# mala-lab/GGAD

Measured on AMD Instinct MI355X. Metric: training nodes/sec (DGraph-Fin mini-batch GGAD), higher is better.
Workload: dtype f32; 1 GPU; DGraph-Fin-size synthetic graph, mini-batch GGAD (GCN encoder); nodes=3700550, directed_entries=72953930, feat=17, emb=64, batch=150+50, graph=powerlaw(alpha=2.1,max_degree=2000), chunk_batches=150, hop2=ldsw, overlap=False, dense_cus=0, chain=0, dense_steps=XCD-resident chunk kernel: one launch per chunk on 28 CUs of one XCD, parallelism=dp1, optimizer=adam(lr=1e-3,wd=0.007), batch_streams=the reference's stream

## Files before the change

ggad_amd/csrc/common.h:

```cpp
#pragma once
#include <hip/hip_runtime.h>
#include <stdint.h>
#include <mutex>
#include "../../include/ggad_hip.h"

#define GGAD_WAVE 64
#define GGAD_MAX_D 64
#define GGAD_MAX_F 1024

void ggad_set_error(hipError_t e, const char *where);

#define GGAD_CHECK_LAUNCH(where)                 \
  do {                                           \
    hipError_t _e = hipGetLastError();           \
    if (_e != hipSuccess) {                      \
      ggad_set_error(_e, where);                 \
      return GGAD_E_LAUNCH;                      \
    }                                            \
  } while (0)

#define GGAD_REQUIRE(cond) \
  do {                     \
    if (!(cond)) return GGAD_E_INVALID; \
  } while (0)
// ... 32 lines not shown

__device__ __forceinline__ void ggad_adam_elem(float &pi, float &mi, float &vi, float g, float wd, float sc0, float sc1) {
  float gi = fmaf(wd, pi, g);
  mi = fmaf(gi - mi, 0.1f, mi);
  vi = fmaf(0.001f * gi, gi, vi * 0.999f);
  const float denom = sqrtf(vi) / sc1 + 1e-8f;
  pi = pi - sc0 * (mi / denom);
}

__device__ __forceinline__ int lower_bound_i32(const int32_t *__restrict__ a, int lo, int hi, int key) {
  while (lo < hi) {
    int mid = (lo + hi) >> 1;
    if (a[mid] < key) lo = mid + 1; else hi = mid;
  }
  return lo;
}

__device__ __forceinline__ bool ggad_vblock(int skip, unsigned &vb, unsigned &vg) {
  const unsigned b = blockIdx.x, n = gridDim.x;
  if (skip < 0) { vb = b; vg = n; return true; }
  const unsigned sk = (unsigned)skip;
  if ((b & 7u) == sk) return false;
  vb = b - ((b >> 3) + ((b & 7u) > sk ? 1u : 0u));
  vg = n - ((n >> 3) + ((n & 7u) > sk ? 1u : 0u));
  return true;
}
static inline unsigned ggad_skip_grid(unsigned want, int skip) { return skip < 0 ? want : (unsigned)(((uint64_t)(want + 1) * 8 + 6) / 7); }

constexpr int GGAD_CTR_STRIDE = 16;
constexpr int GGAD_CTR_GROUPS = 0 * GGAD_CTR_STRIDE, GGAD_CTR_ITEMS = 1 * GGAD_CTR_STRIDE, GGAD_CTR_PART = 2 * GGAD_CTR_STRIDE,
              GGAD_CTR_CURSOR = 3 * GGAD_CTR_STRIDE, GGAD_CTR_PC = 4 * GGAD_CTR_STRIDE,
              GGAD_CTR_BIG = 5 * GGAD_CTR_STRIDE,
              GGAD_CTR_RANGE0 = 6 * GGAD_CTR_STRIDE,
              GGAD_CTR_PROF = 14 * GGAD_CTR_STRIDE;
constexpr int GGAD_RANGES = 8;
constexpr int GGAD_RANGE_DEG = 256;
constexpr int GGAD_PLAN_COUNTERS = 16 * GGAD_CTR_STRIDE;

struct ggad_plan_view {
  const int32_t *batch_ptr, *batch_ent_ptr, *nodes, *row_slot, *ent_ptr, *row_ck_ptr, *ck_rc, *ck_e0;
  int32_t n_batches, n_rows, n_ents, n_chunks;
  int32_t seg_stride;
  int64_t pair_bound;
};
int ggad_int_hop1(const ggad_mb_plan *P, const ggad_plan_view &V, int ldsw, int reset_now, hipStream_t st);
int ggad_int_global_hop2(const ggad_mb_plan *P, const ggad_plan_view &V, hipStream_t st, hipEvent_t ev0, hipEvent_t ev1);
int ggad_int_ldsw_hop2(const ggad_mb_plan *P, const ggad_plan_view &V, hipStream_t st, hipEvent_t ev0, hipEvent_t ev1);
int ggad_int_range_deg();

int ggad_int_gemm_slab(const float *A, const float *B, float *C, int M, int N, int K, int64_t lda, int64_t sbk, int64_t sbn, int64_t ldc,
                       const float *bias, int relu, hipStream_t st, const float *prelu_a = nullptr, float *C2 = nullptr, int64_t ldc2 = 0);

int64_t ggad_int_wgrad_tn_ws(int R, int m, int n);
int ggad_int_wgrad_tn(const float *P, int64_t ldp, const float *Q, int64_t ldq, int R, int m, int n, float *D, float *ws, hipStream_t st,
                      int *vpq = nullptr);

constexpr int GGAD_MB_BWD_PARTS = 256;
struct ggad_xchg_view;
bool ggad_int_wide_ok(int D, int F);
int ggad_int_wide_project(const float *params, int32_t D, int32_t F, const float *x2, const int32_t *ent_own, int32_t ent0,
                          int32_t n_ents, float *h2, ggad_stream_t stream);
int ggad_int_wide_fwd_rows(const float *params, int32_t D, int32_t F, const float *x1, const float *h2, const int32_t *ent_ptr,
                           const int32_t *ent_own, const int32_t *labels, int32_t row0, int32_t n_rows, int32_t ent0, float *h1,
                           float *nbar, float *gen, ggad_stream_t stream);
int ggad_int_wide_loss(const float *params, int32_t D, int32_t F, const float *h1, const float *nbar, const float *gen,
                       const int32_t *labels, const int32_t *pos_meta, const int32_t *row_pos, const int32_t *ent_ptr,
                       int32_t row0, int32_t n_rows, float *loss_ws, float *losses8, float *d_h1, float *d_gen, float *d_nbar,
                       float *dz, float *coef_a, float *coef_g, int32_t *step_counter, ggad_stream_t stream);
int ggad_int_wide_row_coefs(const float *params, int32_t D, int32_t F, const int32_t *labels, const int32_t *ent_ptr,
                            int32_t row0, int32_t n_rows, const float *h1, const float *gen, const float *d_h1,
// ... 29 lines not shown
```

ggad_amd/csrc/hop2_ldsw.hip:

```cpp
#include <algorithm>
#include <atomic>
#include <climits>
#include <mutex>

#include "common.h"

namespace {

#ifdef GGAD_G2_PROF
struct G2Prof { unsigned long long a[8], t; };
#define G2_ARG , G2Prof &prof
#define G2_PASS , prof
#define G2_MARK(i) do { __builtin_amdgcn_sched_barrier(0); __builtin_amdgcn_s_waitcnt(0); const unsigned long long t_ = wall_clock64(); \
                        prof.a[i] += t_ - prof.t; prof.t = t_; __builtin_amdgcn_sched_barrier(0); } while (0)
#define TC_MARK(i) do { __syncthreads(); if (threadIdx.x == 0) { const unsigned long long t_ = wall_clock64(); tcp[i] += t_ - tct; tct = t_; } } while (0)
#else
#define G2_ARG
#define G2_PASS
#define G2_MARK(i)
#define TC_MARK(i)
#endif

constexpr int SLICE = 256;
constexpr int GRP_W = 10;
// ... 503 lines not shown
      for (int q = 0; q < 4; ++q) wa[4 * c + q] = a < G ? wv[q] : 0.0f;
    }
    __builtin_amdgcn_wave_barrier();
    {
      const int ix = min(blk + 64 + lane, last);
      k_nx = col[s + ix];
#pragma unroll
      for (int j = 0; j < G; ++j) c_nx[j] = pc[pb[j] + ix];
    }
    G2_MARK(3);
#pragma unroll
    for (int i = 0; i < 16; ++i) {
      acc0 = __builtin_amdgcn_mfma_f32_16x16x4f32(wa[i], x[i].x, acc0, 0, 0, 0);
      acc1 = __builtin_amdgcn_mfma_f32_16x16x4f32(wa[i], x[i].y, acc1, 0, 0, 0);
    }
    G2_MARK(4);
  }
#pragma unroll
  for (int j = 0; j < G; ++j) {
    const int src = (lane >> 1) + 16 * (j >> 2);
    const float v0 = __shfl(acc0[j & 3], src & 63, GGAD_WAVE), v1 = __shfl(acc1[j & 3], src & 63, GGAD_WAVE);
    tot[j] = (lane & 1) ? v1 : v0;
  }
}

__device__ __forceinline__ int range_tile(int r, int n_tiles) { return (int)(((int64_t)r * n_tiles) / GGAD_RANGES); }

__global__ void __launch_bounds__(256) k_build_groups(const int32_t *__restrict__ ent_own, const int32_t *__restrict__ ent_col,
                                                      const int32_t *__restrict__ own_deg, int n_ents,
                                                      int32_t *__restrict__ node_head, const int32_t *__restrict__ own_next,
                                                      const int32_t *__restrict__ tile_off, int n_tiles,
                                                      int32_t *__restrict__ grp, int32_t *__restrict__ items,
                                                      int32_t *__restrict__ big, int32_t *__restrict__ gbnd,
                                                      int32_t *__restrict__ counters, int range_deg, int skip) {
  unsigned vbx, vgx;
  if (!ggad_vblock(skip, vbx, vgx)) return;
  const int e = vbx * 256 + threadIdx.x;
  const int lane = lane_id();
  int u = 0, m = 0, ng = 0, ns = 0, deg = 0;
  if (e < n_ents && ent_own[e] == e) {
    u = ent_col[e];
    if (node_head[u] == e + 1) {
      for (int cur = e + 1; cur != 0; cur = own_next[cur - 1]) ++m;
      ng = (m + 7) >> 3;
      deg = own_deg[e];
      ns = deg > range_deg ? GGAD_RANGES : (deg > SLICE ? (deg + SLICE - 1) / SLICE : 1);
    }
  }
  const bool is_big = deg > range_deg;
  const int c1 = is_big ? 0 : ng * ns, c2 = ns > 1 ? m * ns : 0, c3 = is_big ? ng : 0;
  int v0 = ng, v1 = c1, v2 = c2, v3 = c3;
#pragma unroll
  for (int off = 1; off < GGAD_WAVE; off <<= 1) {
    const int t0 = __shfl_up(v0, off, GGAD_WAVE), t1 = __shfl_up(v1, off, GGAD_WAVE), t2 = __shfl_up(v2, off, GGAD_WAVE),
              t3 = __shfl_up(v3, off, GGAD_WAVE);
    if (lane >= off) { v0 += t0; v1 += t1; v2 += t2; v3 += t3; }
  }
  __shared__ int wg_tot[4][5];
  const int wid = threadIdx.x >> 6;
  if (lane == GGAD_WAVE - 1) { wg_tot[0][wid] = v0; wg_tot[1][wid] = v1; wg_tot[2][wid] = v2; wg_tot[3][wid] = v3; }
  __syncthreads();
  if (threadIdx.x < 4) {
    const int k = threadIdx.x;
    int sum = 0;
    for (int w = 0; w < 4; ++w) { const int t = wg_tot[k][w]; wg_tot[k][w] = sum; sum += t; }
    int32_t *ctr = counters + (k == 0 ? GGAD_CTR_GROUPS : (k == 1 ? GGAD_CTR_ITEMS : (k == 2 ? GGAD_CTR_PART : GGAD_CTR_BIG)));
    wg_tot[k][4] = sum > 0 ? atomicAdd(ctr, sum) : 0;
  }
  __syncthreads();
  const int b0 = wg_tot[0][4] + wg_tot[0][wid], b1 = wg_tot[1][4] + wg_tot[1][wid], b2 = wg_tot[2][4] + wg_tot[2][wid],
            b3 = wg_tot[3][4] + wg_tot[3][wid];
  if (ng == 0) return;
  const int gbase = b0 + v0 - ng, ibase = b1 + v1 - c1, pbase = b2 + v2 - c2, bbase = b3 + v3 - c3;
  int bnd[GGAD_RANGES + 1];
  if (is_big) {
    const int32_t *row = tile_off + (int64_t)u * (n_tiles + 1);
#pragma unroll
    for (int r = 0; r <= GGAD_RANGES; ++r) bnd[r] = row[range_tile(r, n_tiles)];
  }
  int cur = e + 1;
  for (int g = 0; g < ng; ++g) {
    int32_t *rec = grp + (int64_t)(gbase + g) * GRP_W;
#pragma unroll
    for (int j = 0; j < 8; ++j) {
      int v = -1;
      if (cur != 0) { v = cur - 1; cur = own_next[v]; }
      rec[j] = v;
    }
    rec[8] = pbase + g * 8 * ns;
    rec[9] = ns;
    if (is_big) {
      big[bbase + g] = gbase + g;
      int32_t *bo = gbnd + (int64_t)(bbase + g) * (GGAD_RANGES + 1);
#pragma unroll
      for (int r = 0; r <= GGAD_RANGES; ++r) bo[r] = bnd[r];
    } else {
      for (int sl = 0; sl < ns; ++sl) {
        int32_t *it = items + (int64_t)(ibase + sl * ng + g) * 2;
        it[0] = gbase + g;
        it[1] = sl;
      }
    }
  }
  node_head[u] = 0;
}

template <int FT, bool MF>
__global__ void __launch_bounds__(256) k_gather2_items(const int32_t *__restrict__ col, const float *__restrict__ feat, int F_rt,
                                                       int stride, const int32_t *__restrict__ own_rp,
                                                       const int32_t *__restrict__ own_deg, const int32_t *__restrict__ pw_base,
                                                       const uint16_t *__restrict__ pc, const int32_t *__restrict__ grp,
                                                       const int32_t *__restrict__ items, const int32_t *__restrict__ big,
                                                       const int32_t *__restrict__ gbnd, int32_t *__restrict__ counters,
                                                       float *__restrict__ x2, float *__restrict__ part2, int affine, int take_cap, int skip) {
  static_assert(ITEM_GRAB == 4 && GRP_W <= 10, "lane layout of the metadata loads: 16 lanes per item of a grab (10, 11: range bounds)");
  unsigned vbx, vgx;
  if (!ggad_vblock(skip, vbx, vgx)) return;
  const int F = FT ? FT : F_rt;
  const int lane = lane_id();
  __shared__ __attribute__((aligned(16))) float mf_lds[MF ? 4 * MF_LDS : 4];
  float *lw = mf_lds + (MF ? (threadIdx.x >> 6) * MF_LDS : 0);
  const int n_small = counters[GGAD_CTR_ITEMS], n_big = counters[GGAD_CTR_BIG];
  const int q_l = lane >> 4, r_l = lane & 15;
// ... 81 lines not shown
        else if (n == 2) { float t2[2]; gather_slice_mfma<2>(col, feat, s, n0, n1, inv_sr, n, pb, pc, lane, lw, k_first, t2 G2_PASS); tot[0] = t2[0]; tot[1] = t2[1]; }
        else if (n <= 4) { float t4[4]; gather_slice_mfma<4>(col, feat, s, n0, n1, inv_sr, n, pb, pc, lane, lw, k_first, t4 G2_PASS);
#pragma unroll
          for (int j = 0; j < 4; ++j) tot[j] = t4[j]; }
        else gather_slice_mfma<8>(col, feat, s, n0, n1, inv_sr, n, pb, pc, lane, lw, k_first, tot G2_PASS);
      } else
      if (n == 1) { float t1[1]; gather_slice<1, FT>(col, feat, F, stride, s, n0, n1, inv_sr, n, pb, pc, lane, k_first, t1 G2_PASS); tot[0] = t1[0]; }
      else if (n == 2) { float t2[2]; gather_slice<2, FT>(col, feat, F, stride, s, n0, n1, inv_sr, n, pb, pc, lane, k_first, t2 G2_PASS); tot[0] = t2[0]; tot[1] = t2[1]; }
      else if (n <= 4) { float t4[4]; gather_slice<4, FT>(col, feat, F, stride, s, n0, n1, inv_sr, n, pb, pc, lane, k_first, t4 G2_PASS);
#pragma unroll
        for (int j = 0; j < 4; ++j) tot[j] = t4[j]; }
      else gather_slice<8, FT>(col, feat, F, stride, s, n0, n1, inv_sr, n, pb, pc, lane, k_first, tot G2_PASS);
#pragma unroll
      for (int j = 0; j < 8; ++j) {
        if (j < n && lane < F) {
          if (ns == 1) x2[(int64_t)e[j] * F + lane] = (deg == 0) ? inv_sr * 0.0f : tot[j];
          else part2[((int64_t)pbase + (int64_t)j * ns + sl) * F + lane] = tot[j];
        }
      }
      G2_MARK(5);
    }
    }
  }
  }
#ifdef GGAD_G2_PROF
  if (lane == 0) {
    prof.a[6] = wall_clock64() - t_begin;
    unsigned long long *out = reinterpret_cast<unsigned long long *>(counters + GGAD_CTR_PROF);
    for (int k = 0; k < 7; ++k) atomicAdd(out + k, prof.a[k]);
  }
#endif
}

__global__ void __launch_bounds__(256) k_gather2_combine(const int32_t *__restrict__ grp, const int32_t *__restrict__ counters,
                                                         const float *__restrict__ part2, int F, float *__restrict__ x2, int skip) {
  unsigned vbx, vgx;
  if (!ggad_vblock(skip, vbx, vgx)) return;
  const int lane = lane_id();
  const int n_groups = counters[GGAD_CTR_GROUPS];
  const int rpi = 64 / F;
  const int g = lane / F, f = lane - g * F;
  for (int gi = vbx * 4 + (threadIdx.x >> 6); gi < n_groups; gi += vgx * 4) {
    const int rv = (lane < GRP_W) ? grp[(int64_t)gi * GRP_W + lane] : -1;
    const int ns = __builtin_amdgcn_readlane(rv, 9);
    if (ns <= 1) continue;
    const int pbase = __builtin_amdgcn_readlane(rv, 8);
    for (int j0 = 0; j0 < 8; j0 += rpi) {
      const int j = j0 + g;
      const int ej = __shfl(rv, j & 7, GGAD_WAVE);
      if (g < rpi && j < 8 && ej >= 0) {
        float acc = 0.0f;
#pragma unroll 4
        for (int sl = 0; sl < ns; ++sl) acc += part2[((int64_t)pbase + (int64_t)j * ns + sl) * F + f];
        x2[(int64_t)ej * F + f] = acc;
      }
    }
  }
}

__global__ void __launch_bounds__(256) k_gather2_w(const int32_t *__restrict__ col, const float *__restrict__ feat, int F, int stride,
                                                   const int32_t *__restrict__ ent_own, int n_ents,
                                                   const int32_t *__restrict__ own_rp, const int32_t *__restrict__ own_deg,
                                                   const int32_t *__restrict__ pw_base, const uint16_t *__restrict__ pc,
                                                   float *__restrict__ x2, int skip) {
  unsigned vbx, vgx;
  if (!ggad_vblock(skip, vbx, vgx)) return;
  const int e0 = vbx * 4 + (threadIdx.x >> 6);
  if (e0 >= n_ents || ent_own[e0] != e0) return;
  const int lane = lane_id();
  const int s = own_rp[e0];
  const int deg = own_deg[e0];
  const int pb0 = pw_base[e0];
  const float inv_sr = 1.0f / sqrtf((float)deg);
  if (F <= 64) {
    const int pb[8] = {pb0, 0, 0, 0, 0, 0, 0, 0};
    float total = 0.0f;
#ifdef GGAD_G2_PROF
    G2Prof prof = {};
// ... 47 lines not shown
  const int n_tiles = (int)((P->n_nodes + TW_TILE - 1) >> TW_SHIFT);
  const int skip = P->xcd_skip >= 0 && P->xcd_skip < 8 ? P->xcd_skip : -1;
  const bool tile_major = P->tile_start != nullptr && P->col_t != nullptr;
  k_seg_transpose<<<dim3(ggad_skip_grid((unsigned)((V.n_ents + 63) / 64), skip)), dim3(256), 0, st>>>(
      P->tile_off, tile_major ? P->tile_start : nullptr, n_tiles, P->ent_own, P->ent_col, V.n_ents, V.seg_stride, P->seg_t, skip);
  const size_t lds = (size_t)(TW_TILE / 2) * 4 + (size_t)(3 * TW_MAXOWN + 1) * 4 + (size_t)TW_BRK * 4;
  {
    static std::mutex mu;
    static int state[64] = {};
    int dev = 0;
    if (hipGetDevice(&dev) != hipSuccess || dev < 0 || dev >= 64) return GGAD_E_INVALID;
    std::lock_guard<std::mutex> lock(mu);
    if (state[dev] == 0) {
      const bool ok = hipFuncSetAttribute((const void *)k_tile_counts, hipFuncAttributeMaxDynamicSharedMemorySize, (int)lds) == hipSuccess;
      (void)hipGetLastError();
      state[dev] = ok ? 1 : -1;
    }
    if (state[dev] != 1) { ggad_set_error(hipErrorInvalidValue, "mb_plan_build: this device cannot give k_tile_counts its LDS"); return GGAD_E_LAUNCH; }
  }
  if (P->ev_tile0) (void)hipEventRecord(static_cast<hipEvent_t>(P->ev_tile0), st);
  static const int tc_map = [] { const char *e = getenv("GGAD_TC_MAP"); return e ? atoi(e) : -1; }();
  const bool class_map = tc_map >= 0 ? tc_map != 0 : tile_major;
  const unsigned tc_grid = class_map ? 8u * (unsigned)((n_tiles + (skip < 0 ? 8 : 7) - 1) / (skip < 0 ? 8 : 7)) * (unsigned)V.n_batches
                                      : ggad_skip_grid((unsigned)n_tiles * (unsigned)V.n_batches, skip);
  k_tile_counts<<<dim3(tc_grid), dim3(TW_T), lds, st>>>(tile_major ? P->col_t : P->col, P->seg_t, V.seg_stride, P->own_rp, V.batch_ent_ptr,
                                                        P->pw_base, P->pc, n_tiles, V.n_batches, P->counters, skip, (tile_major ? 1 : 0) | (class_map ? 2 : 0));
  if (P->ev_tile1) (void)hipEventRecord(static_cast<hipEvent_t>(P->ev_tile1), st);
  if (ev0) (void)hipEventRecord(ev0, st);
  const int F = P->feat_dim;
  if (P->node_major && F <= 64) {
    const int range_deg = ggad_int_range_deg();
    static const int affine = [] { const char *e = getenv("GGAD_RANGE_AFFINE"); return e ? atoi(e) : 1; }();
    int32_t *big = P->items + 2 * (int64_t)P->item_cap, *gbnd = P->items + 3 * (int64_t)P->item_cap;
    k_build_groups<<<dim3(ggad_skip_grid((unsigned)((V.n_ents + 255) / 256), skip)), dim3(256), 0, st>>>(
        P->ent_own, P->ent_col, P->own_deg, V.n_ents, P->node_head, P->own_next, P->tile_off, n_tiles, P->grp, P->items, big, gbnd,
        P->counters, range_deg, skip);
    const int64_t max_items = (int64_t)V.n_ents + (V.pair_bound > 0 ? V.pair_bound : P->pair_cap) / SLICE;
    static const int env_wg = [] { const char *e = getenv("GGAD_G2_WG_PER_CU"); return e ? atoi(e) : 0; }();
    static const int env_cap = [] { const char *e = getenv("GGAD_G2_TAKE_CAP"); return e ? atoi(e) : 0; }();
    const bool small_launch = V.n_batches <= 32;
    const int wg_per_cu = env_wg > 0 ? env_wg : (small_launch ? 3 : 4);
    const int take_cap = env_cap > 0 ? env_cap : (small_launch ? 8 : 12);
    const unsigned wgs = (unsigned)std::min<int64_t>((max_items + 4 * ITEM_GRAB - 1) / (4 * ITEM_GRAB), 256 * wg_per_cu);
    if (F == 17 && P->feat_stride == 32 && V.n_batches >= g_mfma_batches.load())
      k_gather2_items<17, true><<<dim3(ggad_skip_grid(wgs, skip)), dim3(256), 0, st>>>(P->col, P->feat, F, P->feat_stride, P->own_rp, P->own_deg,
                                                                                       P->pw_base, P->pc, P->grp, P->items, big, gbnd, P->counters,
                                                                                       P->x2, P->part2, affine, take_cap, skip);
    else if (F == 17)
      k_gather2_items<17, false><<<dim3(ggad_skip_grid(wgs, skip)), dim3(256), 0, st>>>(P->col, P->feat, F, P->feat_stride, P->own_rp, P->own_deg,
                                                                                 P->pw_base, P->pc, P->grp, P->items, big, gbnd, P->counters,
                                                                                 P->x2, P->part2, affine, take_cap, skip);
    else
      k_gather2_items<0, false><<<dim3(ggad_skip_grid(wgs, skip)), dim3(256), 0, st>>>(P->col, P->feat, F, P->feat_stride, P->own_rp, P->own_deg,
                                                                                P->pw_base, P->pc, P->grp, P->items, big, gbnd, P->counters,
                                                                                P->x2, P->part2, affine, take_cap, skip);
    const unsigned cg = (unsigned)std::min<int64_t>(((int64_t)V.n_ents + 3) / 4, 16384);
    k_gather2_combine<<<dim3(ggad_skip_grid(cg, skip)), dim3(256), 0, st>>>(P->grp, P->counters, P->part2, F, P->x2, skip);
  } else {
    k_gather2_w<<<dim3(ggad_skip_grid((unsigned)((V.n_ents + 3) / 4), skip)), dim3(256), 0, st>>>(
        P->col, P->feat, F, P->feat_stride, P->ent_own, V.n_ents, P->own_rp, P->own_deg, P->pw_base, P->pc, P->x2, skip);
  }
  if (ev1) (void)hipEventRecord(ev1, st);
  GGAD_CHECK_LAUNCH("mb_plan_build (ldsw 2-hop)");
  return GGAD_OK;
}

extern "C" {

int ggad_mb_ldsw_tile_shift(void) { return TW_SHIFT; }
int ggad_mb_ldsw_max_owners(void) { return TW_MAXOWN; }
int32_t ggad_mb_slice_len(void) { return SLICE; }
int32_t ggad_mb_group_words(void) { return GRP_W; }
int ggad_mb_set_gather_options(int32_t mfma_min_batches, int32_t range_deg) {
  if (mfma_min_batches >= 0) g_mfma_batches.store(mfma_min_batches);
  if (range_deg >= 0) g_range_deg.store(range_deg);
  return GGAD_OK;
}
int32_t ggad_mb_item_words(void) { return 3 + GGAD_RANGES + 1; }
int32_t ggad_mb_plan_counter_elems(void) { return GGAD_PLAN_COUNTERS; }
int64_t ggad_mb_tile_offsets_elems(int64_t n_nodes, int32_t tile_shift) {
  return n_nodes * (((n_nodes + (1LL << tile_shift) - 1) >> tile_shift) + 1);
}
int64_t ggad_mb_ldsw_seg_elems(int64_t n_nodes, int64_t n_entries_cap) {
  return 2 * (((n_nodes + TW_TILE - 1) >> TW_SHIFT) + 1) * ((n_entries_cap + 63) / 64 * 64);
}

int ggad_mb_tile_offsets(const int32_t *rowptr, const int32_t *col, int64_t n_nodes, int32_t tile_shift, int32_t *tile_off,
                         ggad_stream_t stream) {
  GGAD_REQUIRE(rowptr && col && tile_off && n_nodes >= 0 && tile_shift >= 8 && tile_shift <= 24);
  if (n_nodes == 0) return GGAD_OK;
// ... 32 lines not shown
```

ggad_amd/csrc/plan.hip:

```cpp
#include "common.h"

namespace {

constexpr int SCAN_T = 256;
constexpr int SCAN_ITEMS = 8;
constexpr int SCAN_TILE = SCAN_T * SCAN_ITEMS;

__device__ __forceinline__ int block_exclusive_scan(int v, int *total) {
  __shared__ int wsum[SCAN_T / GGAD_WAVE];
  const int lane = lane_id(), wid = threadIdx.x / GGAD_WAVE;
  int inc = v;
#pragma unroll
  for (int off = 1; off < GGAD_WAVE; off <<= 1) {
    int t = __shfl_up(inc, off, GGAD_WAVE);
    if (lane >= off) inc += t;
  }
  if (lane == GGAD_WAVE - 1) wsum[wid] = inc;
  __syncthreads();
  int base = 0, tot = 0;
#pragma unroll
  for (int w = 0; w < SCAN_T / GGAD_WAVE; ++w) {
    int s = wsum[w];
    if (w < wid) base += s;
    tot += s;
// ... 51 lines not shown
      const int jj = __shfl(j, src & 63, GGAD_WAVE);
      const float ws = __shfl(w, src & 63, GGAD_WAVE);
      ww[u] = (src < count) ? ws : 0.0f;
      x[u] = (lane_active && src < count) ? feat[(int64_t)jj * F + fbase + f] : 0.0f;
    }
#pragma unroll
    for (int u = 0; u < 4; ++u) acc = fmaf(ww[u], x[u], acc);
  }
  for (; t < iters; ++t) {
    const int src = t * rpi + g;
    const int jj = __shfl(j, src & 63, GGAD_WAVE);
    const float ws = __shfl(w, src & 63, GGAD_WAVE);
    const float ww = (src < count) ? ws : 0.0f;
    const float x = (lane_active && src < count) ? feat[(int64_t)jj * F + fbase + f] : 0.0f;
    acc = fmaf(ww, x, acc);
  }
}

__device__ __forceinline__ float reduce_groups(float acc, int F, int rpi) {
  float tot = acc;
  for (int gg = 1; gg < rpi; ++gg) tot += __shfl(acc, (lane_id() + gg * F) & 63, GGAD_WAVE);
  return tot;
}

__global__ void __launch_bounds__(256) k_expand(const int32_t *__restrict__ rowptr, const int32_t *__restrict__ col,
                                                const int32_t *__restrict__ nodes, const int32_t *__restrict__ row_slot,
                                                const int32_t *__restrict__ ent_ptr, const int32_t *__restrict__ ck_rc,
                                                const int32_t *__restrict__ ck_e0, int n_chunks, int64_t n_nodes,
                                                int32_t *__restrict__ ent_col, int32_t *__restrict__ ent_slot,
                                                int32_t *__restrict__ ent_row, int32_t *__restrict__ cnt1,
                                                int32_t *__restrict__ own1, int32_t *__restrict__ counters, int skip) {
  unsigned vbx, vgx;
  if (!ggad_vblock(skip, vbx, vgx)) return;
  if (vbx == 0 && threadIdx.x < GGAD_PLAN_COUNTERS && counters != nullptr) counters[threadIdx.x] = 0;
  const int ck = (int)((vbx * 256u + threadIdx.x) >> 4);
  const int i = threadIdx.x & 15;
  if (ck >= n_chunks) return;
  const int rc = ck_rc[ck];
  if (i >= (rc & 63)) return;
  const int row = rc >> 6;
  const int e = ck_e0[ck] + i;
  const int e_row = ent_ptr[row];
  const int r = ent_ptr[row + 1] - e_row;
  const int idx = e - e_row;
  const int v = nodes[row];
  const int s = rowptr[v];
  const int deg = rowptr[v + 1] - s;
  int j;
  if (r == deg) {
    j = col[s + idx];
  } else {
    const int a = idx > 0 ? col[s + idx - 1] : -1;
    const int b = idx < deg ? col[s + idx] : 0x7fffffff;
    j = (b < v) ? b : (a < v ? v : a);
  }
  const int slot = row_slot[row];
  ent_col[e] = j;
  ent_slot[e] = slot;
  ent_row[e] = row;
  const int64_t soff = (int64_t)slot * n_nodes;
  const int old = atomicAdd(&cnt1[soff + j], 1);
  if (old == 0) own1[soff + j] = e;
}

__global__ void __launch_bounds__(256) k_gather1c(const float *__restrict__ feat, int F, int stride,
                                                  const int32_t *__restrict__ row_slot, const int32_t *__restrict__ ent_ptr,
                                                  const int32_t *__restrict__ row_ck_ptr, const int32_t *__restrict__ ck_rc,
// ... 370 lines not shown
```

ggad_amd/csrc/plan_build.cpp:

```cpp
#include <algorithm>
#include <chrono>
#include <cstdint>
#include <cstdio>
#include <cstdlib>
#include <cstring>
#include <vector>

#include "common.h"

namespace {
inline int64_t align4(int64_t x) { return (x + 3) & ~(int64_t)3; }
}

extern "C" {

int ggad_event_create(int32_t timing, void **out) {
  if (!out) return GGAD_E_INVALID;
  hipEvent_t ev = nullptr;
  const hipError_t e = hipEventCreateWithFlags(&ev, timing ? hipEventDefault : hipEventDisableTiming);
  if (e != hipSuccess) { ggad_set_error(e, "event_create"); return GGAD_E_LAUNCH; }
  *out = ev;
  return GGAD_OK;
}
int ggad_event_destroy(void *event) {
  if (!event) return GGAD_OK;
  const hipError_t e = hipEventDestroy(static_cast<hipEvent_t>(event));
  if (e != hipSuccess) { ggad_set_error(e, "event_destroy"); return GGAD_E_LAUNCH; }
  return GGAD_OK;
}
int ggad_event_record(void *event, ggad_stream_t stream) {
  if (!event) return GGAD_E_INVALID;
  const hipError_t e = hipEventRecord(static_cast<hipEvent_t>(event), as_stream(stream));
  if (e != hipSuccess) { ggad_set_error(e, "event_record"); return GGAD_E_LAUNCH; }
  return GGAD_OK;
}
int ggad_event_synchronize(void *event) {
  if (!event) return GGAD_E_INVALID;
  const hipError_t e = hipEventSynchronize(static_cast<hipEvent_t>(event));
  if (e != hipSuccess) { ggad_set_error(e, "event_synchronize"); return GGAD_E_LAUNCH; }
  return GGAD_OK;
}
int ggad_event_elapsed_ms(void *start, void *stop, float *ms_host) {
  if (!start || !stop || !ms_host) return GGAD_E_INVALID;
  const hipError_t e = hipEventElapsedTime(ms_host, static_cast<hipEvent_t>(start), static_cast<hipEvent_t>(stop));
  if (e != hipSuccess) { ggad_set_error(e, "event_elapsed_ms"); return GGAD_E_LAUNCH; }
  return GGAD_OK;
}

int ggad_mb_plan_build(const ggad_mb_plan *P, const int64_t *nodes_host, const int32_t *batch_ptr_host, int32_t n_batches,
                       const int64_t *labels_host, ggad_mb_plan_info *info, int64_t *ent_ptr_host_out,
                       int64_t *batch_ent_ptr_host_out, int32_t *batch_max_row_host_out, ggad_stream_t stream) {
  GGAD_REQUIRE(P && nodes_host && batch_ptr_host && info);
  GGAD_REQUIRE(P->rowptr && P->col && P->feat && P->closed_deg_host && P->stage_host && P->stage && P->stage_event);
  GGAD_REQUIRE(P->cnt1 && P->own1 && P->ent_col && P->ent_slot && P->ent_row && P->ent_own && P->ent_c1 && P->x1 && P->ck_part);
  GGAD_REQUIRE(P->feat_dim >= 1 && P->feat_dim <= GGAD_MAX_F && P->feat_stride >= P->feat_dim && P->n_nodes >= 1);
  GGAD_REQUIRE(P->ck_part_stride >= (P->feat_dim < 64 ? 64 : P->feat_dim));
  GGAD_REQUIRE(n_batches >= 1 && n_batches <= P->max_batches && batch_ptr_host[0] == 0);
  const bool train = P->train != 0;
  if (train) GGAD_REQUIRE(labels_host && P->x2 && (P->hop2 == 1 || P->hop2 == 2));
  std::memset(info, 0, sizeof(*info));
  static const bool timing = getenv("GGAD_BUILD_TIMING") != nullptr;
  const auto tt0 = std::chrono::steady_clock::now();
  const int nb = n_batches;
  const int64_t rows = batch_ptr_host[nb];
  GGAD_REQUIRE(rows >= 1 && rows < (1 << 25));
  for (int b = 0; b < nb; ++b) GGAD_REQUIRE(batch_ptr_host[b + 1] > batch_ptr_host[b]);
  const int CL = 16;
  const int SL = ggad_mb_slice_len();

  int64_t n_ents = 0, n_chunks = 0, bound = 0;
  int64_t max_batch_ents = 0;
  const bool want_ldsw = train && P->hop2 == 1;
  if (want_ldsw) GGAD_REQUIRE(P->pair_bound_host && P->tile_off && P->own_deg && P->own_rp && P->pw_base && P->node_head &&
                              P->own_next && P->grp && P->counters);
  static thread_local std::vector<int32_t> row_deg;
  if ((int64_t)row_deg.size() < rows) row_deg.resize((size_t)rows);
  constexpr int PF = 24;
  const int64_t *pack = P->node_pack_host;
  constexpr int64_t PACK_MASK = (1LL << 40) - 1;
  for (int64_t i = 0; i < rows && i < PF; ++i) {
    const int64_t v = nodes_host[i];
    GGAD_REQUIRE(v >= 0 && v < P->n_nodes);
    if (pack) { __builtin_prefetch(&pack[v]); continue; }
    __builtin_prefetch(&P->closed_deg_host[v]);
    if (want_ldsw) __builtin_prefetch(&P->pair_bound_host[v]);
  }
  for (int b = 0; b < nb; ++b) {
    int64_t be = 0;
    for (int64_t i = batch_ptr_host[b]; i < batch_ptr_host[b + 1]; ++i) {
      if (i + PF < rows) {
        const int64_t vn = nodes_host[i + PF];
        GGAD_REQUIRE(vn >= 0 && vn < P->n_nodes);
        if (pack) __builtin_prefetch(&pack[vn]);
        else {
          __builtin_prefetch(&P->closed_deg_host[vn]);
          if (want_ldsw) __builtin_prefetch(&P->pair_bound_host[vn]);
        }
      }
      const int64_t v = nodes_host[i];
      const int64_t pk = pack ? pack[v] : 0;
      const int64_t r = pack ? (pk >> 40) : P->closed_deg_host[v];
      row_deg[(size_t)i] = (int32_t)r;
      be += r;
      n_chunks += (r + CL - 1) / CL;
      if (want_ldsw) bound += pack ? (pk & PACK_MASK) : P->pair_bound_host[v];
    }
    n_ents += be;
    max_batch_ents = std::max(max_batch_ents, be);
  }
  GGAD_REQUIRE(n_ents < (1LL << 31) - 1);
  int mode = train ? P->hop2 : 0;
  if (mode == 1 && (max_batch_ents >= 65536 || bound >= (1LL << 31) - 1 || P->n_nodes * (int64_t)P->feat_stride * 4 >= (1LL << 32)))
    mode = 2;
  const int64_t off_bp = 0, off_bep = align4(nb + 1), off_nodes = off_bep + align4(nb + 1), off_labels = off_nodes + align4(rows),
                off_meta = off_labels + align4(rows), off_rpos = off_meta + align4(rows), off_slot = off_rpos + align4(rows),
                off_eptr = off_slot + align4(rows), off_ckp = off_eptr + align4(rows + 1), off_ckrc = off_ckp + align4(rows + 1),
                off_cke0 = off_ckrc + align4(n_chunks), stage_need = off_cke0 + align4(n_chunks);
  const int64_t seg_stride = (n_ents + 63) / 64 * 64;
  const int64_t n_tiles1 = ((P->n_nodes + (1LL << ggad_mb_ldsw_tile_shift()) - 1) >> ggad_mb_ldsw_tile_shift()) + 1;
  info->pair_bound = bound;
  info->n_batches = nb;
  info->n_rows = (int32_t)rows;
  info->n_ents = (int32_t)n_ents;
  info->n_chunks = (int32_t)n_chunks;
  info->mode = mode;
  info->off_batch_ptr = off_bp; info->off_batch_ent_ptr = off_bep; info->off_nodes = off_nodes; info->off_labels = off_labels;
  info->off_pos_meta = off_meta; info->off_row_pos = off_rpos; info->off_row_slot = off_slot; info->off_ent_ptr = off_eptr;
  info->off_row_ck_ptr = off_ckp; info->off_ck_rc = off_ckrc; info->off_ck_e0 = off_cke0;
  info->need_rows = rows; info->need_ents = n_ents; info->need_chunks = n_chunks; info->need_stage = stage_need;
  if (mode == 1) {
    info->need_pairs = bound;
    info->need_items = n_ents + bound / SL;
    info->need_part2 = (2 + (ggad_int_range_deg() == INT32_MAX ? 0 : (int64_t)GGAD_RANGES * SL / GGAD_RANGE_DEG)) * (bound / SL) + 8;
    info->need_seg = ((P->tile_start && P->col_t) ? 2 : 1) * n_tiles1 * seg_stride;
  }
  info->need_cnt2 = (mode == 2 && P->cnt2 == nullptr) ? 1 : 0;
  if (rows > P->rows_cap || n_ents > P->ent_cap || n_chunks > P->ck_cap || stage_need > P->stage_cap || info->need_cnt2 ||
      (mode == 1 && (info->need_pairs > P->pair_cap || info->need_items > P->item_cap || info->need_part2 > P->part2_cap ||
                     info->need_seg > P->seg_cap)))
    return GGAD_E_CAPACITY;
  if (mode == 1) GGAD_REQUIRE(P->seg_t && P->pc && P->items && P->part2);

  const auto tt1 = std::chrono::steady_clock::now();
  hipStream_t st = as_stream(stream);
  hipError_t he = hipEventSynchronize(static_cast<hipEvent_t>(P->stage_event));
  if (he != hipSuccess) { ggad_set_error(he, "mb_plan_build (stage event)"); return GGAD_E_LAUNCH; }
  const auto tt2 = std::chrono::steady_clock::now();
  int32_t *S = P->stage_host;
  int32_t *bp = S + off_bp, *bep = S + off_bep, *nd = S + off_nodes, *lb = S + off_labels, *meta = S + off_meta,
          *rpos = S + off_rpos, *slot = S + off_slot, *eptr = S + off_eptr, *ckp = S + off_ckp, *ckrc = S + off_ckrc,
          *cke0 = S + off_cke0;
  int64_t e = 0, c = 0;
  for (int b = 0; b < nb; ++b) {
    const int r0 = batch_ptr_host[b], r1 = batch_ptr_host[b + 1];
    bp[b] = r0;
    bep[b] = (int32_t)e;
    if (batch_ent_ptr_host_out) batch_ent_ptr_host_out[b] = e;
    int max_r = 0;
    for (int i = r0; i < r1; ++i) {
      const int32_t v = (int32_t)nodes_host[i];
      const int r = row_deg[(size_t)i];
      nd[i] = v;
      slot[i] = b;
      eptr[i] = (int32_t)e;
      ckp[i] = (int32_t)c;
      if (ent_ptr_host_out) ent_ptr_host_out[i] = e;
      for (int k = 0; k < r; k += CL) {
        ckrc[c] = (i << 6) | std::min(CL, r - k);
        cke0[c] = (int32_t)(e + k);
        ++c;
      }
      e += r;
      max_r = std::max(max_r, r);
    }
    if (batch_max_row_host_out) batch_max_row_host_out[b] = max_r;
    if (train) {
      int q = 0;
      for (int pass = 0; pass < 2; ++pass)
        for (int i = r0; i < r1; ++i) {
          const int64_t l = labels_host[i];
          if (l != 0 && l != 1) return GGAD_E_INVALID;
          if ((int)l != pass) continue;
          meta[r0 + q] = (i << 2) | ((int)l << 1);
          rpos[i] = q;
          ++q;
        }
      for (int i = r0; i < r1; ++i) {
        lb[i] = (int32_t)labels_host[i];
        meta[i] |= (int32_t)labels_host[i];
      }
    }
  }
  bp[nb] = (int32_t)rows;
  bep[nb] = (int32_t)e;
  eptr[rows] = (int32_t)e;
  ckp[rows] = (int32_t)c;
  if (batch_ent_ptr_host_out) batch_ent_ptr_host_out[nb] = e;
  if (ent_ptr_host_out) ent_ptr_host_out[rows] = e;
  const auto tt3 = std::chrono::steady_clock::now();
  he = hipMemcpyAsync(P->stage, S, (size_t)stage_need * sizeof(int32_t), hipMemcpyHostToDevice, st);
  if (he != hipSuccess) { ggad_set_error(he, "mb_plan_build (upload)"); return GGAD_E_LAUNCH; }
  he = hipEventRecord(static_cast<hipEvent_t>(P->stage_event), st);
  if (he != hipSuccess) { ggad_set_error(he, "mb_plan_build (stage event record)"); return GGAD_E_LAUNCH; }

  const auto tt4 = std::chrono::steady_clock::now();
  ggad_plan_view V;
  const int32_t *D = P->stage;
  V.batch_ptr = D + off_bp; V.batch_ent_ptr = D + off_bep; V.nodes = D + off_nodes; V.row_slot = D + off_slot;
  V.ent_ptr = D + off_eptr; V.row_ck_ptr = D + off_ckp; V.ck_rc = D + off_ckrc; V.ck_e0 = D + off_cke0;
  V.n_batches = nb; V.n_rows = (int32_t)rows; V.n_ents = (int32_t)n_ents; V.n_chunks = (int32_t)n_chunks;
  V.seg_stride = (int32_t)seg_stride;
  V.pair_bound = bound;
  int rc = ggad_int_hop1(P, V, mode == 1 ? 1 : 0, mode != 2 ? 1 : 0, st);
  if (rc) return rc;
  hipEvent_t ev0 = static_cast<hipEvent_t>(P->ev_gather0), ev1 = static_cast<hipEvent_t>(P->ev_gather1);
  if (mode == 1) rc = ggad_int_ldsw_hop2(P, V, st, ev0, ev1);
  else if (mode == 2) rc = ggad_int_global_hop2(P, V, st, ev0, ev1);
  if (timing) {
    const auto tt5 = std::chrono::steady_clock::now();
    auto us = [](auto a, auto b) { return std::chrono::duration<double, std::micro>(b - a).count(); };
    fprintf(stderr, "[ggad_mb_plan_build] %d batches: sizes %.1f  stage-event wait %.1f  fill %.1f  copy + event %.1f  launches %.1f us (%lld KB staged)\n", nb,
            us(tt0, tt1), us(tt1, tt2), us(tt2, tt3), us(tt3, tt4), us(tt4, tt5), (long long)(stage_need * 4 / 1024));
  }
  return rc;
}

}
```

Measured before the change: 3.326 million nodes/s.

## Fuse host plan size pass with fill and compact multi-slice combine list

The host plan builder now computes per-row degrees and writes the structural tables in one pass after waiting on the stage event, instead of a size pass followed by a fill pass. Chunk start offsets go to a provisional far location and are moved into place once the chunk count is known. Label partitioning also changes from two scans to a count-then-place pass. On the GPU, group building now records a compact list of groups split across several slices, so the combine kernel walks only those on a smaller grid rather than scanning every group and skipping single-slice ones. The trade-offs are an extra counter slot and item-buffer region, a memmove on the host, and the stage-event wait now happening before the size computation.

```diff
diff --git a/ggad_amd/csrc/common.h b/ggad_amd/csrc/common.h
--- a/ggad_amd/csrc/common.h
+++ b/ggad_amd/csrc/common.h
@@ -88,10 +88,11 @@
               GGAD_CTR_CURSOR = 3 * GGAD_CTR_STRIDE, GGAD_CTR_PC = 4 * GGAD_CTR_STRIDE,
               GGAD_CTR_BIG = 5 * GGAD_CTR_STRIDE,
               GGAD_CTR_RANGE0 = 6 * GGAD_CTR_STRIDE,
-              GGAD_CTR_PROF = 14 * GGAD_CTR_STRIDE;
+              GGAD_CTR_PROF = 14 * GGAD_CTR_STRIDE,
+              GGAD_CTR_MULTI = 16 * GGAD_CTR_STRIDE;
 constexpr int GGAD_RANGES = 8;
 constexpr int GGAD_RANGE_DEG = 256;
-constexpr int GGAD_PLAN_COUNTERS = 16 * GGAD_CTR_STRIDE;
+constexpr int GGAD_PLAN_COUNTERS = 17 * GGAD_CTR_STRIDE;
 
 struct ggad_plan_view {
   const int32_t *batch_ptr, *batch_ent_ptr, *nodes, *row_slot, *ent_ptr, *row_ck_ptr, *ck_rc, *ck_e0;
diff --git a/ggad_amd/csrc/hop2_ldsw.hip b/ggad_amd/csrc/hop2_ldsw.hip
--- a/ggad_amd/csrc/hop2_ldsw.hip
+++ b/ggad_amd/csrc/hop2_ldsw.hip
@@ -559,7 +559,8 @@
                                                       const int32_t *__restrict__ tile_off, int n_tiles,
                                                       int32_t *__restrict__ grp, int32_t *__restrict__ items,
                                                       int32_t *__restrict__ big, int32_t *__restrict__ gbnd,
-                                                      int32_t *__restrict__ counters, int range_deg, int skip) {
+                                                      int32_t *__restrict__ multi, int32_t *__restrict__ counters, int range_deg,
+                                                      int skip) {
   unsigned vbx, vgx;
   if (!ggad_vblock(skip, vbx, vgx)) return;
   const int e = vbx * 256 + threadIdx.x;
@@ -576,29 +577,30 @@
   }
   const bool is_big = deg > range_deg;
   const int c1 = is_big ? 0 : ng * ns, c2 = ns > 1 ? m * ns : 0, c3 = is_big ? ng : 0;
-  int v0 = ng, v1 = c1, v2 = c2, v3 = c3;
+  const int c4 = ns > 1 ? ng : 0;
+  int v0 = ng, v1 = c1, v2 = c2, v3 = c3, v4 = c4;
 #pragma unroll
   for (int off = 1; off < GGAD_WAVE; off <<= 1) {
     const int t0 = __shfl_up(v0, off, GGAD_WAVE), t1 = __shfl_up(v1, off, GGAD_WAVE), t2 = __shfl_up(v2, off, GGAD_WAVE),
-              t3 = __shfl_up(v3, off, GGAD_WAVE);
-    if (lane >= off) { v0 += t0; v1 += t1; v2 += t2; v3 += t3; }
-  }
-  __shared__ int wg_tot[4][5];
+              t3 = __shfl_up(v3, off, GGAD_WAVE), t4 = __shfl_up(v4, off, GGAD_WAVE);
+    if (lane >= off) { v0 += t0; v1 += t1; v2 += t2; v3 += t3; v4 += t4; }
+  }
+  __shared__ int wg_tot[5][5];
   const int wid = threadIdx.x >> 6;
-  if (lane == GGAD_WAVE - 1) { wg_tot[0][wid] = v0; wg_tot[1][wid] = v1; wg_tot[2][wid] = v2; wg_tot[3][wid] = v3; }
+  if (lane == GGAD_WAVE - 1) { wg_tot[0][wid] = v0; wg_tot[1][wid] = v1; wg_tot[2][wid] = v2; wg_tot[3][wid] = v3; wg_tot[4][wid] = v4; }
   __syncthreads();
-  if (threadIdx.x < 4) {
+  if (threadIdx.x < 5) {
     const int k = threadIdx.x;
     int sum = 0;
     for (int w = 0; w < 4; ++w) { const int t = wg_tot[k][w]; wg_tot[k][w] = sum; sum += t; }
-    int32_t *ctr = counters + (k == 0 ? GGAD_CTR_GROUPS : (k == 1 ? GGAD_CTR_ITEMS : (k == 2 ? GGAD_CTR_PART : GGAD_CTR_BIG)));
+    int32_t *ctr = counters + (k == 0 ? GGAD_CTR_GROUPS : (k == 1 ? GGAD_CTR_ITEMS : (k == 2 ? GGAD_CTR_PART : (k == 3 ? GGAD_CTR_BIG : GGAD_CTR_MULTI))));
     wg_tot[k][4] = sum > 0 ? atomicAdd(ctr, sum) : 0;
   }
   __syncthreads();
   const int b0 = wg_tot[0][4] + wg_tot[0][wid], b1 = wg_tot[1][4] + wg_tot[1][wid], b2 = wg_tot[2][4] + wg_tot[2][wid],
-            b3 = wg_tot[3][4] + wg_tot[3][wid];
+            b3 = wg_tot[3][4] + wg_tot[3][wid], b4 = wg_tot[4][4] + wg_tot[4][wid];
   if (ng == 0) return;
-  const int gbase = b0 + v0 - ng, ibase = b1 + v1 - c1, pbase = b2 + v2 - c2, bbase = b3 + v3 - c3;
+  const int gbase = b0 + v0 - ng, ibase = b1 + v1 - c1, pbase = b2 + v2 - c2, bbase = b3 + v3 - c3, mbase = b4 + v4 - c4;
   int bnd[GGAD_RANGES + 1];
   if (is_big) {
     const int32_t *row = tile_off + (int64_t)u * (n_tiles + 1);
@@ -616,6 +618,7 @@
     }
     rec[8] = pbase + g * 8 * ns;
     rec[9] = ns;
+    if (ns > 1) multi[mbase + g] = gbase + g;
     if (is_big) {
       big[bbase + g] = gbase + g;
       int32_t *bo = gbnd + (int64_t)(bbase + g) * (GGAD_RANGES + 1);
@@ -763,18 +766,21 @@
 #endif
 }
 
-__global__ void __launch_bounds__(256) k_gather2_combine(const int32_t *__restrict__ grp, const int32_t *__restrict__ counters,
-                                                         const float *__restrict__ part2, int F, float *__restrict__ x2, int skip) {
+__global__ void __launch_bounds__(256) k_gather2_combine(const int32_t *__restrict__ grp, const int32_t *__restrict__ multi,
+                                                         const int32_t *__restrict__ counters, const float *__restrict__ part2, int F,
+                                                         float *__restrict__ x2, int skip) {
   unsigned vbx, vgx;
   if (!ggad_vblock(skip, vbx, vgx)) return;
+  const int n_multi = counters[GGAD_CTR_MULTI];
+  const int w0 = vbx * 4 + (threadIdx.x >> 6);
+  if (w0 >= n_multi) return;
   const int lane = lane_id();
-  const int n_groups = counters[GGAD_CTR_GROUPS];
   const int rpi = 64 / F;
   const int g = lane / F, f = lane - g * F;
-  for (int gi = vbx * 4 + (threadIdx.x >> 6); gi < n_groups; gi += vgx * 4) {
+  for (int mi = w0; mi < n_multi; mi += vgx * 4) {
+    const int gi = multi[mi];
     const int rv = (lane < GRP_W) ? grp[(int64_t)gi * GRP_W + lane] : -1;
     const int ns = __builtin_amdgcn_readlane(rv, 9);
-    if (ns <= 1) continue;
     const int pbase = __builtin_amdgcn_readlane(rv, 8);
     for (int j0 = 0; j0 < 8; j0 += rpi) {
       const int j = j0 + g;
@@ -888,9 +894,10 @@
     const int range_deg = ggad_int_range_deg();
     static const int affine = [] { const char *e = getenv("GGAD_RANGE_AFFINE"); return e ? atoi(e) : 1; }();
     int32_t *big = P->items + 2 * (int64_t)P->item_cap, *gbnd = P->items + 3 * (int64_t)P->item_cap;
+    int32_t *multi = P->items + (int64_t)(3 + GGAD_RANGES) * P->item_cap;
     k_build_groups<<<dim3(ggad_skip_grid((unsigned)((V.n_ents + 255) / 256), skip)), dim3(256), 0, st>>>(
         P->ent_own, P->ent_col, P->own_deg, V.n_ents, P->node_head, P->own_next, P->tile_off, n_tiles, P->grp, P->items, big, gbnd,
-        P->counters, range_deg, skip);
+        multi, P->counters, range_deg, skip);
     const int64_t max_items = (int64_t)V.n_ents + (V.pair_bound > 0 ? V.pair_bound : P->pair_cap) / SLICE;
     static const int env_wg = [] { const char *e = getenv("GGAD_G2_WG_PER_CU"); return e ? atoi(e) : 0; }();
     static const int env_cap = [] { const char *e = getenv("GGAD_G2_TAKE_CAP"); return e ? atoi(e) : 0; }();
@@ -910,8 +917,9 @@
       k_gather2_items<0, false><<<dim3(ggad_skip_grid(wgs, skip)), dim3(256), 0, st>>>(P->col, P->feat, F, P->feat_stride, P->own_rp, P->own_deg,
                                                                                 P->pw_base, P->pc, P->grp, P->items, big, gbnd, P->counters,
                                                                                 P->x2, P->part2, affine, take_cap, skip);
-    const unsigned cg = (unsigned)std::min<int64_t>(((int64_t)V.n_ents + 3) / 4, 16384);
-    k_gather2_combine<<<dim3(ggad_skip_grid(cg, skip)), dim3(256), 0, st>>>(P->grp, P->counters, P->part2, F, P->x2, skip);
+    const int64_t max_multi = std::min<int64_t>(V.n_ents, (V.pair_bound > 0 ? V.pair_bound : P->pair_cap) / SLICE);
+    const unsigned cg = (unsigned)std::max<int64_t>(1, std::min<int64_t>((max_multi + 3) / 4, 2048));
+    k_gather2_combine<<<dim3(ggad_skip_grid(cg, skip)), dim3(256), 0, st>>>(P->grp, multi, P->counters, P->part2, F, P->x2, skip);
   } else {
     k_gather2_w<<<dim3(ggad_skip_grid((unsigned)((V.n_ents + 3) / 4), skip)), dim3(256), 0, st>>>(
         P->col, P->feat, F, P->feat_stride, P->ent_own, V.n_ents, P->own_rp, P->own_deg, P->pw_base, P->pc, P->x2, skip);
diff --git a/ggad_amd/csrc/plan.hip b/ggad_amd/csrc/plan.hip
--- a/ggad_amd/csrc/plan.hip
+++ b/ggad_amd/csrc/plan.hip
@@ -107,7 +107,8 @@
                                                 int32_t *__restrict__ own1, int32_t *__restrict__ counters, int skip) {
   unsigned vbx, vgx;
   if (!ggad_vblock(skip, vbx, vgx)) return;
-  if (vbx == 0 && threadIdx.x < GGAD_PLAN_COUNTERS && counters != nullptr) counters[threadIdx.x] = 0;
+  if (vbx == 0 && counters != nullptr)
+    for (int i = threadIdx.x; i < GGAD_PLAN_COUNTERS; i += 256) counters[i] = 0;
   const int ck = (int)((vbx * 256u + threadIdx.x) >> 4);
   const int i = threadIdx.x & 15;
   if (ck >= n_chunks) return;
diff --git a/ggad_amd/csrc/plan_build.cpp b/ggad_amd/csrc/plan_build.cpp
--- a/ggad_amd/csrc/plan_build.cpp
+++ b/ggad_amd/csrc/plan_build.cpp
@@ -10,6 +10,90 @@
 
 namespace {
 inline int64_t align4(int64_t x) { return (x + 3) & ~(int64_t)3; }
+
+constexpr int CL = 16;
+constexpr int PF = 24;
+constexpr int64_t PACK_MASK = (1LL << 40) - 1;
+
+struct RowTables {
+  int32_t *bp, *bep, *nd, *slot, *eptr, *ckp, *ckrc, *cke0;
+  int64_t piece_cap;
+  int64_t *ent_ptr_out, *batch_ent_ptr_out;
+  int32_t *batch_max_row_out;
+};
+struct RowTotals {
+  int64_t n_ents = 0, n_chunks = 0, bound = 0, max_batch_ents = 0;
+  bool bad_node = false;
+};
+
+template <bool FILL>
+RowTotals walk_rows(const ggad_mb_plan *P, const int64_t *nodes_host, const int32_t *batch_ptr_host, int nb, bool want_ldsw,
+                    const RowTables &T) {
+  RowTotals R;
+  const int64_t rows = batch_ptr_host[nb];
+  const int64_t *pack = P->node_pack_host;
+  auto request = [&](int64_t v) {
+    if (pack) { __builtin_prefetch(&pack[v]); return; }
+    __builtin_prefetch(&P->closed_deg_host[v]);
+    if (want_ldsw) __builtin_prefetch(&P->pair_bound_host[v]);
+  };
+  for (int64_t i = 0; i < rows && i < PF; ++i) {
+    const int64_t v = nodes_host[i];
+    if (v < 0 || v >= P->n_nodes) { R.bad_node = true; return R; }
+    request(v);
+  }
+  int64_t e = 0, c = 0;
+  for (int b = 0; b < nb; ++b) {
+    const int r0 = batch_ptr_host[b], r1 = batch_ptr_host[b + 1];
+    const int64_t e_batch = e;
+    if (FILL) {
+      T.bp[b] = r0;
+      T.bep[b] = (int32_t)e;
+      if (T.batch_ent_ptr_out) T.batch_ent_ptr_out[b] = e;
+    }
+    int max_r = 0;
+    for (int i = r0; i < r1; ++i) {
+      if (i + PF < rows) {
+        const int64_t vn = nodes_host[i + PF];
+        if (vn < 0 || vn >= P->n_nodes) { R.bad_node = true; return R; }
+        request(vn);
+      }
+      const int64_t v = nodes_host[i];
+      const int64_t pk = pack ? pack[v] : 0;
+      const int r = (int)(pack ? (pk >> 40) : P->closed_deg_host[v]);
+      if (want_ldsw) R.bound += pack ? (pk & PACK_MASK) : P->pair_bound_host[v];
+      const int np = (r + CL - 1) / CL;
+      if (FILL) {
+        T.nd[i] = (int32_t)v;
+        T.slot[i] = b;
+        T.eptr[i] = (int32_t)e;
+        T.ckp[i] = (int32_t)c;
+        if (T.ent_ptr_out) T.ent_ptr_out[i] = e;
+        if (c + np <= T.piece_cap)
+          for (int k = 0, cc = (int)c; k < r; k += CL, ++cc) {
+            T.ckrc[cc] = (i << 6) | std::min(CL, r - k);
+            T.cke0[cc] = (int32_t)(e + k);
+          }
+        max_r = std::max(max_r, r);
+      }
+      c += np;
+      e += r;
+    }
+    if (FILL && T.batch_max_row_out) T.batch_max_row_out[b] = max_r;
+    R.max_batch_ents = std::max(R.max_batch_ents, e - e_batch);
+  }
+  if (FILL) {
+    T.bp[nb] = (int32_t)rows;
+    T.bep[nb] = (int32_t)e;
+    T.eptr[rows] = (int32_t)e;
+    T.ckp[rows] = (int32_t)c;
+    if (T.batch_ent_ptr_out) T.batch_ent_ptr_out[nb] = e;
+    if (T.ent_ptr_out) T.ent_ptr_out[rows] = e;
+  }
+  R.n_ents = e;
+  R.n_chunks = c;
+  return R;
+}
 }
 
 extern "C" {
@@ -65,57 +149,35 @@
   const int64_t rows = batch_ptr_host[nb];
   GGAD_REQUIRE(rows >= 1 && rows < (1 << 25));
   for (int b = 0; b < nb; ++b) GGAD_REQUIRE(batch_ptr_host[b + 1] > batch_ptr_host[b]);
-  const int CL = 16;
   const int SL = ggad_mb_slice_len();
-
-  int64_t n_ents = 0, n_chunks = 0, bound = 0;
-  int64_t max_batch_ents = 0;
   const bool want_ldsw = train && P->hop2 == 1;
   if (want_ldsw) GGAD_REQUIRE(P->pair_bound_host && P->tile_off && P->own_deg && P->own_rp && P->pw_base && P->node_head &&
                               P->own_next && P->grp && P->counters);
-  static thread_local std::vector<int32_t> row_deg;
-  if ((int64_t)row_deg.size() < rows) row_deg.resize((size_t)rows);
-  constexpr int PF = 24;
-  const int64_t *pack = P->node_pack_host;
-  constexpr int64_t PACK_MASK = (1LL << 40) - 1;
-  for (int64_t i = 0; i < rows && i < PF; ++i) {
-    const int64_t v = nodes_host[i];
-    GGAD_REQUIRE(v >= 0 && v < P->n_nodes);
-    if (pack) { __builtin_prefetch(&pack[v]); continue; }
-    __builtin_prefetch(&P->closed_deg_host[v]);
-    if (want_ldsw) __builtin_prefetch(&P->pair_bound_host[v]);
-  }
-  for (int b = 0; b < nb; ++b) {
-    int64_t be = 0;
-    for (int64_t i = batch_ptr_host[b]; i < batch_ptr_host[b + 1]; ++i) {
-      if (i + PF < rows) {
-        const int64_t vn = nodes_host[i + PF];
-        GGAD_REQUIRE(vn >= 0 && vn < P->n_nodes);
-        if (pack) __builtin_prefetch(&pack[vn]);
-        else {
-          __builtin_prefetch(&P->closed_deg_host[vn]);
-          if (want_ldsw) __builtin_prefetch(&P->pair_bound_host[vn]);
-        }
-      }
-      const int64_t v = nodes_host[i];
-      const int64_t pk = pack ? pack[v] : 0;
-      const int64_t r = pack ? (pk >> 40) : P->closed_deg_host[v];
-      row_deg[(size_t)i] = (int32_t)r;
-      be += r;
-      n_chunks += (r + CL - 1) / CL;
-      if (want_ldsw) bound += pack ? (pk & PACK_MASK) : P->pair_bound_host[v];
-    }
-    n_ents += be;
-    max_batch_ents = std::max(max_batch_ents, be);
-  }
+
+  const int64_t off_labels = 0, off_meta = align4(rows), off_rpos = off_meta + align4(rows), off_bp = off_rpos + align4(rows),
+                off_bep = off_bp + align4(nb + 1), off_nodes = off_bep + align4(nb + 1), off_slot = off_nodes + align4(rows),
+                off_eptr = off_slot + align4(rows), off_ckp = off_eptr + align4(rows + 1), off_ckrc = off_ckp + align4(rows + 1);
+  const int64_t piece_cap = std::max<int64_t>(0, std::min<int64_t>(align4(P->ck_cap), ((P->stage_cap - off_ckrc) / 2) & ~(int64_t)3));
+  const int64_t off_cke0_far = off_ckrc + piece_cap;
+  const bool can_fill = rows <= P->rows_cap && off_ckrc <= P->stage_cap;
+
+  hipStream_t st = as_stream(stream);
+  hipError_t he = hipEventSynchronize(static_cast<hipEvent_t>(P->stage_event));
+  if (he != hipSuccess) { ggad_set_error(he, "mb_plan_build (stage event)"); return GGAD_E_LAUNCH; }
+  const auto tt1 = std::chrono::steady_clock::now();
+
+  int32_t *S = P->stage_host;
+  RowTables T = {S + off_bp, S + off_bep, S + off_nodes, S + off_slot, S + off_eptr, S + off_ckp, S + off_ckrc, S + off_cke0_far, piece_cap,
+                 ent_ptr_host_out, batch_ent_ptr_host_out, batch_max_row_host_out};
+  const RowTotals R = can_fill ? walk_rows<true>(P, nodes_host, batch_ptr_host, nb, want_ldsw, T)
+                               : walk_rows<false>(P, nodes_host, batch_ptr_host, nb, want_ldsw, T);
+  GGAD_REQUIRE(!R.bad_node);
+  const int64_t n_ents = R.n_ents, n_chunks = R.n_chunks, bound = R.bound;
   GGAD_REQUIRE(n_ents < (1LL << 31) - 1);
   int mode = train ? P->hop2 : 0;
-  if (mode == 1 && (max_batch_ents >= 65536 || bound >= (1LL << 31) - 1 || P->n_nodes * (int64_t)P->feat_stride * 4 >= (1LL << 32)))
+  if (mode == 1 && (R.max_batch_ents >= 65536 || bound >= (1LL << 31) - 1 || P->n_nodes * (int64_t)P->feat_stride * 4 >= (1LL << 32)))
     mode = 2;
-  const int64_t off_bp = 0, off_bep = align4(nb + 1), off_nodes = off_bep + align4(nb + 1), off_labels = off_nodes + align4(rows),
-                off_meta = off_labels + align4(rows), off_rpos = off_meta + align4(rows), off_slot = off_rpos + align4(rows),
-                off_eptr = off_slot + align4(rows), off_ckp = off_eptr + align4(rows + 1), off_ckrc = off_ckp + align4(rows + 1),
-                off_cke0 = off_ckrc + align4(n_chunks), stage_need = off_cke0 + align4(n_chunks);
+  const int64_t off_cke0 = off_ckrc + align4(n_chunks), stage_need = off_cke0 + align4(n_chunks);
   const int64_t seg_stride = (n_ents + 63) / 64 * 64;
   const int64_t n_tiles1 = ((P->n_nodes + (1LL << ggad_mb_ldsw_tile_shift()) - 1) >> ggad_mb_ldsw_tile_shift()) + 1;
   info->pair_bound = bound;
@@ -135,68 +197,37 @@
     info->need_seg = ((P->tile_start && P->col_t) ? 2 : 1) * n_tiles1 * seg_stride;
   }
   info->need_cnt2 = (mode == 2 && P->cnt2 == nullptr) ? 1 : 0;
-  if (rows > P->rows_cap || n_ents > P->ent_cap || n_chunks > P->ck_cap || stage_need > P->stage_cap || info->need_cnt2 ||
+  if (rows > P->rows_cap || n_ents > P->ent_cap || n_chunks > P->ck_cap || stage_need > P->stage_cap || n_chunks > piece_cap ||
+      info->need_cnt2 ||
       (mode == 1 && (info->need_pairs > P->pair_cap || info->need_items > P->item_cap || info->need_part2 > P->part2_cap ||
                      info->need_seg > P->seg_cap)))
     return GGAD_E_CAPACITY;
   if (mode == 1) GGAD_REQUIRE(P->seg_t && P->pc && P->items && P->part2);
-
-  const auto tt1 = std::chrono::steady_clock::now();
-  hipStream_t st = as_stream(stream);
-  hipError_t he = hipEventSynchronize(static_cast<hipEvent_t>(P->stage_event));
-  if (he != hipSuccess) { ggad_set_error(he, "mb_plan_build (stage event)"); return GGAD_E_LAUNCH; }
+  if (off_cke0 != off_cke0_far) std::memmove(S + off_cke0, S + off_cke0_far, (size_t)n_chunks * sizeof(int32_t));
+
   const auto tt2 = std::chrono::steady_clock::now();
-  int32_t *S = P->stage_host;
-  int32_t *bp = S + off_bp, *bep = S + off_bep, *nd = S + off_nodes, *lb = S + off_labels, *meta = S + off_meta,
-          *rpos = S + off_rpos, *slot = S + off_slot, *eptr = S + off_eptr, *ckp = S + off_ckp, *ckrc = S + off_ckrc,
-          *cke0 = S + off_cke0;
-  int64_t e = 0, c = 0;
-  for (int b = 0; b < nb; ++b) {
-    const int r0 = batch_ptr_host[b], r1 = batch_ptr_host[b + 1];
-    bp[b] = r0;
-    bep[b] = (int32_t)e;
-    if (batch_ent_ptr_host_out) batch_ent_ptr_host_out[b] = e;
-    int max_r = 0;
-    for (int i = r0; i < r1; ++i) {
-      const int32_t v = (int32_t)nodes_host[i];
-      const int r = row_deg[(size_t)i];
-      nd[i] = v;
-      slot[i] = b;
-      eptr[i] = (int32_t)e;
-      ckp[i] = (int32_t)c;
-      if (ent_ptr_host_out) ent_ptr_host_out[i] = e;
-      for (int k = 0; k < r; k += CL) {
-        ckrc[c] = (i << 6) | std::min(CL, r - k);
-        cke0[c] = (int32_t)(e + k);
-        ++c;
-      }
-      e += r;
-      max_r = std::max(max_r, r);
+  if (train) {
+    int32_t *lb = S + off_labels, *meta = S + off_meta, *rpos = S + off_rpos;
+    for (int b = 0; b < nb; ++b) {
+      const int r0 = batch_ptr_host[b], r1 = batch_ptr_host[b + 1];
+      int n0 = 0;
+      for (int i = r0; i < r1; ++i) {
+        const int64_t l = labels_host[i];
+        if (l != 0 && l != 1) return GGAD_E_INVALID;
+        lb[i] = (int32_t)l;
+        n0 += l == 0;
+      }
+      int q0 = 0, q1 = n0;
+      for (int i = r0; i < r1; ++i) {
+        const int l = lb[i];
+        const int q = l ? q1++ : q0++;
+        meta[r0 + q] = (i << 2) | (l << 1);
+        rpos[i] = q;
+      }
+      for (int i = r0; i < r1; ++i) meta[i] |= lb[i];
     }
-    if (batch_max_row_host_out) batch_max_row_host_out[b] = max_r;
-    if (train) {
-      int q = 0;
-      for (int pass = 0; pass < 2; ++pass)
-        for (int i = r0; i < r1; ++i) {
-          const int64_t l = labels_host[i];
-          if (l != 0 && l != 1) return GGAD_E_INVALID;
-          if ((int)l != pass) continue;
-          meta[r0 + q] = (i << 2) | ((int)l << 1);
-          rpos[i] = q;
-          ++q;
-        }
-      for (int i = r0; i < r1; ++i) {
-        lb[i] = (int32_t)labels_host[i];
-        meta[i] |= (int32_t)labels_host[i];
-      }
-    }
-  }
-  bp[nb] = (int32_t)rows;
-  bep[nb] = (int32_t)e;
-  eptr[rows] = (int32_t)e;
-  ckp[rows] = (int32_t)c;
-  if (batch_ent_ptr_host_out) batch_ent_ptr_host_out[nb] = e;
-  if (ent_ptr_host_out) ent_ptr_host_out[rows] = e;
+  }
+
   const auto tt3 = std::chrono::steady_clock::now();
   he = hipMemcpyAsync(P->stage, S, (size_t)stage_need * sizeof(int32_t), hipMemcpyHostToDevice, st);
   if (he != hipSuccess) { ggad_set_error(he, "mb_plan_build (upload)"); return GGAD_E_LAUNCH; }
@@ -219,7 +250,8 @@
   if (timing) {
     const auto tt5 = std::chrono::steady_clock::now();
     auto us = [](auto a, auto b) { return std::chrono::duration<double, std::micro>(b - a).count(); };
-    fprintf(stderr, "[ggad_mb_plan_build] %d batches: sizes %.1f  stage-event wait %.1f  fill %.1f  copy + event %.1f  launches %.1f us (%lld KB staged)\n", nb,
+    fprintf(stderr, "[ggad_mb_plan_build] %d batches: stage-event wait %.1f  sizes + structural fill %.1f  labels %.1f  copy + event %.1f  "
+                    "launches %.1f us (%lld KB staged)\n", nb,
             us(tt0, tt1), us(tt1, tt2), us(tt2, tt3), us(tt3, tt4), us(tt4, tt5), (long long)(stage_need * 4 / 1024));
   }
   return rc;
```

After: 3.318 million nodes/s. No clear change (-0.2%).
